# EnterpriseCV-6/Season-NeRF

Measured on AMD Instinct MI355X. Metric: ray-samples/sec (4096 rays x 96 samples forward render, T_NeRF 8x256), higher is better.
Workload: dtype i8x3 (16-bit fixed point as two int8 digits on v_mfma_i32_32x32x32_i8, exact int32 accumulate, fp32 epilogue)

## Files before the change

### season_nerf_amd/csrc/kernels.hip

```cpp
#include "mlp_bf16_device.h"

namespace snerf {


template <int NB, int KS0, int KS1, bool SIN, int TERMS = 3, bool LO_OUT = true>
__device__ __forceinline__ void run_layer(Ring& rg, const uint8_t* stream, uint32_t stream_bytes, lds_char* lds,
                                          lds_cfloat* bias_l, const Frag* in0, const Frag* in1, Frag* out,
                                          f32x16* raw, int wave, int lane) {
    constexpr int KS = KS0 + KS1, NP = NB * KS;
    constexpr bool PIPE = KS >= 4;
    const int h = lane >> 5;
    u32x4 fh[PF], fl[PF] = {};
#pragma unroll
    for (int q = 0; q < PF; ++q) {
        if (q < NP) {
            if (q % kChunkPairs == 0) ring_step(rg, stream, stream_bytes, lds, wave, lane);
            lds_char* ap = lds + rg.cur + (q % kChunkPairs) * kPairBytes + lane * 16;
            fh[q] = *(lds_cu32x4*)ap;
            if (TERMS == 3) fl[q] = *(lds_cu32x4*)(ap + kFragBytes);
        }
    }
    f32x16 accs[2];
    EpiTmp et[8];
    f32x16 next_init = load_bias(bias_l, 0, h);
// ... 113 lines not shown
        const int64_t nc = valid ? n : A.n - 1;
        const int64_t g = VARIANT == 3 ? 0 : nc / A.group_size;

        if constexpr (PROG == PROG_FIELD) {
            float x0, x1, x2;
            if constexpr (VARIANT == 3) raysum_point(rs, A, tile, 4, wave, pass, lane, x0, x1, x2);
            else field_point(A, nc, x0, x1, x2);
            float s0, s1, s2, pcls[C_MAX];
            field_tile_inputs<VARIANT>(A, g, s0, s1, s2, pcls);
            Frag pe[PEPOS_KS];
            make_pe_pos(x0, x1, x2, h, pe);

            constexpr int KW = W / 16, KW2 = W2 / 16;
            Frag hA[KW], hB[KW], x1f[KW2];
            f32x16 raw;
#define LAYER(L, NBv, K0, K1, SINv, IN0, IN1, OUT, RAW)                                                              \
    run_layer<NBv, K0, K1, SINv, (FAST && L != F_FC1) ? 1 : 3, !FAST>(rg, A.stream, A.stream_bytes, lds,                   \
                                 bias_lds + prog_bias_start(PROG_FIELD, W, C_MAX, L), IN0, IN1, OUT, RAW, wave, lane)
            FIELD_TRUNK(LAYER, pe, hA, hB, x1f, raw);
            const float col_r = raw[0], col_g = raw[1], col_b = raw[2], rho_raw = raw[3];
            float sv_raw = 0.f;
            float adj[3 * C_MAX];
#pragma unroll
            for (int i = 0; i < 3 * C_MAX; ++i) adj[i] = 0.f;
            if constexpr (VARIANT <= 1) {
                Frag ps[PESUN_KS];
                make_pe_sun(s0, s1, s2, h, ps);
                Frag sA[KW2], sB[KW2];
                FIELD_SOLAR(LAYER, x1f, ps, sA, sB, raw);
                sv_raw = raw[0];
            }
            if constexpr (VARIANT == 0) {
                FIELD_ADJUST(LAYER, x1f, hA, hB, raw);
#pragma unroll
                for (int i = 0; i < 3 * C_MAX; ++i) adj[i] = raw[i];
            }
#undef LAYER
            if constexpr (VARIANT == 3) {
                RAYSUM_PASS_END(rs, A, tile, pass, passes, 4, wave, wave, 4, true, lane, rho_raw, x0, x1, x2, bias_lds + A.bias_floats);
            } else {
                if (h == 0 && valid) store_field_outputs<VARIANT>(A.out, n, C, x0, x1, x2, col_r, col_g, col_b, rho_raw, sv_raw, adj, pcls);
                tile += gridDim.x;
            }
        } else {
            constexpr int KW = W / 16, W4P = pad32(W / 4), KW4 = W4P / 16;
            f32x16 raw;
#define LAYER(L, NBv, K0, K1, SINv, IN0, IN1, OUT, RAW)                                                              \
    run_layer<NBv, K0, K1, SINv>(rg, A.stream, A.stream_bytes, lds, bias_lds + prog_bias_start(PROG_GROUP, W, C_MAX, L), \
                                 IN0, IN1, OUT, RAW, wave, lane)
            const float t0 = A.time[nc * 4], t1 = A.time[nc * 4 + 1];
            const float s0 = A.sun[nc * 3], s1 = A.sun[nc * 3 + 1], s2 = A.sun[nc * 3 + 2];
            Frag pt[PETIME_KS];
            make_pe_time(t0, t1, h, pt);
            Frag hA[KW], hB[KW];
            LAYER(G_T1, W / 32, PETIME_KS, 0, true, pt, nullptr, hA, nullptr);
            LAYER(G_T2, W / 32, KW, 0, true, hA, nullptr, hB, nullptr);
            LAYER(G_CL, 1, KW, 0, false, hB, nullptr, nullptr, &raw);
            float logit[C_MAX];
#pragma unroll
            for (int c = 0; c < C_MAX; ++c) logit[c] = raw[c];
            Frag ps[PESUN_KS];
            make_pe_sun(s0, s1, s2, h, ps);
            Frag kA[KW4];
            LAYER(G_K1, W4P / 32, PESUN_KS, 0, true, ps, nullptr, kA, nullptr);
            LAYER(G_K2, 1, KW4, 0, false, kA, nullptr, nullptr, &raw);
#undef LAYER
            if (h == 0 && valid) {
                float m = -3.0e38f;
#pragma unroll
                for (int c = 0; c < C_MAX; ++c) if (c < C) m = fmaxf(m, logit[c]);
                float e[C_MAX], sum = 0.f;
#pragma unroll
                for (int c = 0; c < C_MAX; ++c) { e[c] = c < C ? expf(logit[c] - m) : 0.f; sum += e[c]; }
#pragma unroll
                for (int c = 0; c < C_MAX; ++c) if (c < C && A.g_classes) A.g_classes[n * C + c] = e[c] / sum;
#pragma unroll
                for (int k = 0; k < 3; ++k) {
                    if (A.g_sky_raw) A.g_sky_raw[n * 3 + k] = raw[k];
                    if (A.g_sky) A.g_sky[n * 3 + k] = sigmoid_f(raw[k]);
                }
            }
            tile += gridDim.x;
        }
    }
    asm volatile("s_waitcnt vmcnt(0)" ::: "memory");
}

__host__ __device__ constexpr int sun_walk_lds_extra() { return kMaxWalkSuns * 3 * 4; }

__device__ __attribute__((noinline)) void store_softplus(float* p, float x) { *p = softplus_f(x); }

template <int W>
__global__ __launch_bounds__(256, 1) void sun_walk_kernel(const SunWalkArgs SA) {
    const MlpArgs& A = SA.m;
    constexpr int C_MAX = kMaxClasses;
    constexpr int W2 = W / 2;
    const int C = A.n_classes;
    const int n_suns = SA.n_suns;
    FIELD_PROLOGUE(A,
        __attribute__((address_space(3))) float* sun_lds = (__attribute__((address_space(3))) float*)(lds + RING_BYTES + A.bias_floats * 4 + kVoteBytes);
        for (int i = threadIdx.x; i < 3 * n_suns; i += 256) sun_lds[i] = A.sun[i];)

    const int64_t n_tiles = field_tiles(A.n, 0, TILE_PTS, 4);
    snerf_field_out_dev once = A.out;
    once.solar_vis = nullptr;
    once.rho = nullptr;
    for (int64_t tile = blockIdx.x; tile < n_tiles; tile += gridDim.x) {
        const int64_t n = tile * TILE_PTS + wave * 32 + (lane & 31);
        const bool valid = n < A.n;
        const int64_t nc = valid ? n : A.n - 1;
        float x0, x1, x2;
        field_point(A, nc, x0, x1, x2);
        float u0, u1, u2, pcls[C_MAX];
        field_tile_inputs<0>(A, 0, u0, u1, u2, pcls);
        Frag pe[PEPOS_KS];
        make_pe_pos(x0, x1, x2, h, pe);

        constexpr int KW = W / 16, KW2 = W2 / 16;
        Frag hA[KW], hB[KW], x1f[KW2];
        f32x16 raw;
        FIELD_TRUNK(FIELD_LAYER, pe, hA, hB, x1f, raw);
        const float col_r = raw[0], col_g = raw[1], col_b = raw[2], rho_raw = raw[3];
        for (int j = 0; j < n_suns; ++j) {
            const float s0 = sun_lds[3 * j], s1 = sun_lds[3 * j + 1], s2 = sun_lds[3 * j + 2];
            Frag ps[PESUN_KS];
            make_pe_sun(s0, s1, s2, h, ps);
            Frag sA[KW2], sB[KW2];
            FIELD_SOLAR(FIELD_LAYER, x1f, ps, sA, sB, raw);
            if (h == 0 && valid && A.out.solar_vis) A.out.solar_vis[(int64_t)j * A.n + n] = sigmoid_f(raw[0]);
        }
        FIELD_ADJUST(FIELD_LAYER, x1f, hA, hB, raw);
        float adj[3 * C_MAX];
#pragma unroll
        for (int i = 0; i < 3 * C_MAX; ++i) adj[i] = raw[i];
        if (h == 0 && valid) {
            if (A.out.rho) store_softplus(A.out.rho + n, rho_raw);
            store_field_outputs<0>(once, n, C, x0, x1, x2, col_r, col_g, col_b, rho_raw, 0.f, adj, pcls);
        }
    }
    asm volatile("s_waitcnt vmcnt(0)" ::: "memory");
}

__global__ __launch_bounds__(256) void composite_kernel(const CompArgs A) {
    const int lane = threadIdx.x & 63;
    const int64_t r = (int64_t)blockIdx.x * 4 + (threadIdx.x >> 6);
    if (r >= A.n_rays) return;
    const int S = A.n_samples;
    const float tx = A.top[r * 3], ty = A.top[r * 3 + 1], tz = A.top[r * 3 + 2];
    const float bx = A.bot[r * 3], by = A.bot[r * 3 + 1], bz = A.bot[r * 3 + 2];
    const float delta_ray = ray_delta(tx, ty, tz, bx, by, bz, S);
    const bool classic = A.flags & 1, zero_oob = A.flags & 2;
    const float sky0 = A.sky[r * 3], sky1 = A.sky[r * 3 + 1], sky2 = A.sky[r * 3 + 2];

    float carry = 0.f, carry_m = 0.f;
    float a0 = 0.f, a1 = 0.f, a2 = 0.f, svsum = 0.f, acc = 0.f, l0 = 0.f, l1 = 0.f, l2 = 0.f, dist = 0.f;
    float c0 = 0.f, c1 = 0.f, c2 = 0.f;
    float m0 = 0.f, m1 = 0.f, m2 = 0.f;
    float ma0 = 0.f, ma1 = 0.f, ma2 = 0.f;
    for (int base = 0; base < S; base += 64) {
        const int s = base + lane;
        const bool in = s < S;
        const int64_t idx = r * S + (in ? s : S - 1);
        float px, py, pz;
        ray_point(tx, ty, tz, bx, by, bz, A.tvals[in ? s : S - 1], px, py, pz);
        float delta = delta_ray;
        if (zero_oob && outside_cube(px, py, pz)) delta = 0.f;
        const float rho = in ? A.rho[idx] : 0.f;
        const float y = in ? rho * delta : 0.f;
        const RayStep st = transmit_step(y, in, lane, carry);
        carry = st.carry;
        const float pv = st.pv, pe = st.pe, ps = st.ps;
        const float sv = in ? A.solar_vis[idx] : 0.f;
        const float k0 = in ? A.col[idx * 3] : 0.f, k1 = in ? A.col[idx * 3 + 1] : 0.f, k2 = in ? A.col[idx * 3 + 2] : 0.f;
        if (in) {
            if (A.out.pv) A.out.pv[idx] = pv;
            if (A.out.pe) A.out.pe[idx] = pe;
            if (A.out.ps) A.out.ps[idx] = ps;
            if (A.out.delta) A.out.delta[idx] = delta;
        }
        a0 += ps * k0; a1 += ps * k1; a2 += ps * k2;
        svsum += ps * sv;
        acc += ps;
        l0 += ps * px; l1 += ps * py; l2 += ps * pz;
        dist += ps * (delta_ray * (float)(s + 1));
        if (classic) {
            c0 += ps * k0 * (sv + (1.f - sv) * sky0);
            c1 += ps * k1 * (sv + (1.f - sv) * sky1);
            c2 += ps * k2 * (sv + (1.f - sv) * sky2);
        }
        if (A.rho_prior) {
            const float tr = A.trust_dev ? A.trust_dev[0] : A.trust;
            const float rm = in ? (rho * tr + A.rho_prior[idx] * (1.f - tr)) : 0.f;
            const float ym = rm * delta;
            const RayStep stm = transmit_step(ym, in, lane, carry_m);
            carry_m = stm.carry;
            const float psm = stm.ps;
            if (classic) {
                m0 += psm * k0 * (sv + (1.f - sv) * sky0);
                m1 += psm * k1 * (sv + (1.f - sv) * sky1);
                m2 += psm * k2 * (sv + (1.f - sv) * sky2);
                ma0 += psm * k0; ma1 += psm * k1; ma2 += psm * k2;
            } else {
                m0 += psm * k0; m1 += psm * k1; m2 += psm * k2;
            }
        }
    }
    a0 = wave_sum(a0); a1 = wave_sum(a1); a2 = wave_sum(a2);
    svsum = wave_sum(svsum); acc = wave_sum(acc);
    l0 = wave_sum(l0); l1 = wave_sum(l1); l2 = wave_sum(l2); dist = wave_sum(dist);
    if (classic) { c0 = wave_sum(c0); c1 = wave_sum(c1); c2 = wave_sum(c2); }
    if (A.rho_prior) { m0 = wave_sum(m0); m1 = wave_sum(m1); m2 = wave_sum(m2); }
    if (A.rho_prior && classic) { ma0 = wave_sum(ma0); ma1 = wave_sum(ma1); ma2 = wave_sum(ma2); }
    if (lane == 0) {
        const float sv3 = sigmoid_f((svsum - 0.2f) * 30.f);
        const float f0 = sv3 + (1.f - sv3) * sky0, f1 = sv3 + (1.f - sv3) * sky1, f2 = sv3 + (1.f - sv3) * sky2;
        float r0, r1, r2, al0 = a0, al1 = a1, al2 = a2;
        if (A.rho_prior) {
            if (classic) { r0 = m0; r1 = m1; r2 = m2; al0 = ma0; al1 = ma1; al2 = ma2; } else { r0 = m0 * f0; r1 = m1 * f1; r2 = m2 * f2; al0 = m0; al1 = m1; al2 = m2; }
        } else if (classic) { r0 = c0; r1 = c1; r2 = c2; }
        else { r0 = a0 * f0; r1 = a1 * f1; r2 = a2 * f2; }
        if (A.out.rgb) { A.out.rgb[r * 3] = r0; A.out.rgb[r * 3 + 1] = r1; A.out.rgb[r * 3 + 2] = r2; }
        if (A.out.albedo) { A.out.albedo[r * 3] = al0; A.out.albedo[r * 3 + 1] = al1; A.out.albedo[r * 3 + 2] = al2; }
        if (A.out.shadow) A.out.shadow[r] = svsum;
        if (A.out.acc) A.out.acc[r] = acc;
        if (A.out.surf_loc) {
            A.out.surf_loc[r * 3] = l0 / (acc + 1e-8f); A.out.surf_loc[r * 3 + 1] = l1 / (acc + 1e-8f); A.out.surf_loc[r * 3 + 2] = l2 / (acc + 1e-8f);
        }
        if (A.out.surf_dist) A.out.surf_dist[r] = dist / acc;
    }
}

constexpr int T_CHUNK = 12;
__device__ __forceinline__ float sigmoid_fast(float x) { return __builtin_amdgcn_rcpf(1.f + __builtin_amdgcn_exp2f(x * -1.44269504088896341f)); }
template <bool CLASSIC>
__global__ __launch_bounds__(256) void sweep_kernel(const SweepArgs A) {
    constexpr int TH = T_CHUNK / 2;
    const int lane = threadIdx.x & 63, sl = lane & 31, half = lane >> 5;
    const int64_t r = (int64_t)blockIdx.x * 4 + (threadIdx.x >> 6);
    if (r >= A.n_rays) return;
    const int S = A.n_samples, C = A.n_classes;
    const bool explicit_delta = A.deltas != nullptr;
    float tx = 0.f, ty = 0.f, tz = 0.f, bx = 0.f, by = 0.f, bz = 0.f, delta_ray = 0.f;
    if (!explicit_delta) {
        tx = A.top[r * 3]; ty = A.top[r * 3 + 1]; tz = A.top[r * 3 + 2];
        bx = A.bot[r * 3]; by = A.bot[r * 3 + 1]; bz = A.bot[r * 3 + 2];
        const float dx = tx - bx, dy = ty - by, dz = tz - bz;
        delta_ray = __fdiv_rn(__fsqrt_rn(__fadd_rn(__fadd_rn(__fmul_rn(dx, dx), __fmul_rn(dy, dy)), __fmul_rn(dz, dz))), (float)S);
    }
    const bool zero_oob = (A.flags & 2) && !explicit_delta;
    const float sky0 = A.sky[0], sky1 = A.sky[1], sky2 = A.sky[2];
    struct In { float rho, sv, dl, k[3], ad[kMaxClasses][3]; };
    auto fetch = [&](int base) {
        In v;
        const int s = base + sl;
        const int64_t idx = r * S + (s < S ? s : S - 1);
        v.rho = A.rho[idx];
        v.sv = A.solar_vis[idx];
        v.dl = explicit_delta ? A.deltas[idx] : (zero_oob ? A.tvals[s < S ? s : S - 1] : 0.f);
#pragma unroll
        for (int k = 0; k < 3; ++k) v.k[k] = A.col_raw[idx * 3 + k];
        if (A.adjust_vec4 && kMaxClasses >= 4) {
            const float4* p = reinterpret_cast<const float4*>(A.adjust + idx * 12);
            const float4 q0 = p[0], q1 = p[1], q2 = p[2];
            const float f[12] = {q0.x, q0.y, q0.z, q0.w, q1.x, q1.y, q1.z, q1.w, q2.x, q2.y, q2.z, q2.w};
#pragma unroll
            for (int c = 0; c < kMaxClasses; ++c)
#pragma unroll
                for (int k = 0; k < 3; ++k) v.ad[c][k] = c < 4 ? f[c * 3 + k] : 0.f;
            return v;
        }
#pragma unroll
        for (int c = 0; c < kMaxClasses; ++c)
#pragma unroll
            for (int k = 0; k < 3; ++k) v.ad[c][k] = c < C ? A.adjust[(idx * C + c) * 3 + k] : 0.f;
        return v;
    };
    auto half_sum = [](float v) {
#pragma unroll
        for (int o = 16; o > 0; o >>= 1) v += __shfl_xor(v, o, 64);
        return v;
    };
    for (int t0 = 0; t0 < A.n_times; t0 += T_CHUNK) {
        const int tb = t0 + half * TH;
        float cw[TH][kMaxClasses];
#pragma unroll
        for (int t = 0; t < TH; ++t)
#pragma unroll
            for (int c = 0; c < kMaxClasses; ++c) cw[t][c] = (tb + t < A.n_times && c < C) ? A.class_vecs[(tb + t) * C + c] : 0.f;
        float acc[TH][3];
        float accc[CLASSIC ? TH : 1][3];
#pragma unroll
        for (int t = 0; t < TH; ++t) acc[t][0] = acc[t][1] = acc[t][2] = 0.f;
#pragma unroll
        for (int t = 0; t < (CLASSIC ? TH : 1); ++t) accc[t][0] = accc[t][1] = accc[t][2] = 0.f;
        float carry = 0.f, svsum = 0.f, b0 = 0.f, b1 = 0.f, b2 = 0.f;
        In nxt = fetch(0);
        for (int base = 0; base < S; base += 32) {
            const In cur = nxt;
            if (base + 32 < S) nxt = fetch(base + 32);
            const int s = base + sl;
            const bool in = s < S;
            float delta = delta_ray;
            if (explicit_delta) {
                delta = cur.dl;
            } else if (zero_oob) {
                const float tt = cur.dl, omt = __fsub_rn(1.f, tt);
                const float px = __fadd_rn(__fmul_rn(tx, omt), __fmul_rn(bx, tt));
                const float py = __fadd_rn(__fmul_rn(ty, omt), __fmul_rn(by, tt));
                const float pz = __fadd_rn(__fmul_rn(tz, omt), __fmul_rn(bz, tt));
                if (px > 1.f || px < -1.f || py > 1.f || py < -1.f || pz > 1.f || pz < -1.f) delta = 0.f;
            }
            const float y = in ? cur.rho * delta : 0.f;
            float incl = y;
#pragma unroll
            for (int o = 1; o < 32; o <<= 1) {
                const float t = __shfl_up(incl, o, 32);
                if (sl >= o) incl += t;
            }
            const float below = __shfl_up(incl, 1, 32);
            const float excl = carry + (sl == 0 ? 0.f : below);
            carry += __shfl(incl, 31, 32);
            const float ps = in ? expf(-excl) * (1.f - expf(-y)) : 0.f;
            const float sv = in ? cur.sv : 0.f;
            svsum += ps * sv;
            const float k0 = cur.k[0], k1 = cur.k[1], k2 = cur.k[2];
            b0 += ps * sigmoid_fast(k0); b1 += ps * sigmoid_fast(k1); b2 += ps * sigmoid_fast(k2);
#pragma unroll
            for (int t = 0; t < TH; ++t) {
                float m0 = 0.f, m1 = 0.f, m2 = 0.f;
#pragma unroll
                for (int c = 0; c < kMaxClasses; ++c) { m0 += cw[t][c] * cur.ad[c][0]; m1 += cw[t][c] * cur.ad[c][1]; m2 += cw[t][c] * cur.ad[c][2]; }
                const float q0 = ps * sigmoid_fast(k0 + m0), q1 = ps * sigmoid_fast(k1 + m1), q2 = ps * sigmoid_fast(k2 + m2);
                acc[t][0] += q0; acc[t][1] += q1; acc[t][2] += q2;
                if constexpr (CLASSIC) {
                    accc[t][0] += q0 * (sv + (1.f - sv) * sky0);
                    accc[t][1] += q1 * (sv + (1.f - sv) * sky1);
                    accc[t][2] += q2 * (sv + (1.f - sv) * sky2);
                }
            }
        }
        svsum = half_sum(svsum);
        b0 = half_sum(b0); b1 = half_sum(b1); b2 = half_sum(b2);
        const float mask = sigmoid_f((svsum - 0.2f) * 30.f);
        const float f0 = mask + (1.f - mask) * sky0, f1 = mask + (1.f - mask) * sky1, f2 = mask + (1.f - mask) * sky2;
#pragma unroll
        for (int t = 0; t < TH; ++t) {
            const float v0 = half_sum(acc[t][0]), v1 = half_sum(acc[t][1]), v2 = half_sum(acc[t][2]);
            float c0 = 0.f, c1 = 0.f, c2 = 0.f;
            if constexpr (CLASSIC) { c0 = half_sum(accc[t][0]); c1 = half_sum(accc[t][1]); c2 = half_sum(accc[t][2]); }
            if (sl == 0 && tb + t < A.n_times) {
                const int64_t o = ((int64_t)(tb + t) * A.n_rays + r) * 3;
                if (A.season) { A.season[o] = v0; A.season[o + 1] = v1; A.season[o + 2] = v2; }
                if (A.shaded) { A.shaded[o] = v0 * f0; A.shaded[o + 1] = v1 * f1; A.shaded[o + 2] = v2 * f2; }
                if constexpr (CLASSIC) { A.classic[o] = c0; A.classic[o + 1] = c1; A.classic[o + 2] = c2; }
            }
        }
        if (lane == 0 && t0 == 0) {
            if (A.raw_shadow) A.raw_shadow[r] = svsum;
            if (A.shadow_adjust) { A.shadow_adjust[r * 3] = f0; A.shadow_adjust[r * 3 + 1] = f1; A.shadow_adjust[r * 3 + 2] = f2; }
            if (A.base) { A.base[r * 3] = b0; A.base[r * 3 + 1] = b1; A.base[r * 3 + 2] = b2; }
        }
    }
}

hipError_t launch_sweep(const SweepArgs& a, hipStream_t st) {
// ... 426 lines not shown
```

### season_nerf_amd/csrc/kernels_i8x2.hip

```cpp
#include <type_traits>

#include "mlp_i8_device.h"

namespace snerf {

constexpr int NW2 = 8;
constexpr int TILE2 = 32 * NW2;
constexpr int DMA_WAVES2 = 4, PIECES4 = kChunkBytes / kFragBytes / DMA_WAVES2;
constexpr int RING2_D = 7;
constexpr int PFX = 2;
static_assert(PIECES4 == 4 && kChunkPairs == 8, "dma_chunk4 moves four pieces per loading wave; barrier positions assume 8-pair chunks");

struct Ring2 {
    uint32_t wr;
    uint32_t goff;
    uint32_t cur;
};
__device__ __forceinline__ uint32_t ring2_next(uint32_t off) {
    off += kChunkBytes;
    return off == RING2_D * kChunkBytes ? 0u : off;
}
__device__ __forceinline__ void dma_chunk4(const uint8_t* stream, uint32_t goff, lds_char* lds, uint32_t wr, int wave, int lane) {
    const uint8_t* b0 = stream + goff + wave * (4 * kFragBytes);
    const uint32_t dst = (uint32_t)(uintptr_t)(lds + wr + wave * (4 * kFragBytes));
    const uint32_t voff = lane * 16;
    uint32_t keep;
    asm volatile(
        "s_mov_b32 %0, m0\n\t"
        "s_mov_b32 m0, %2\n\t"
        "s_nop 0\n\t"
        "global_load_lds_dwordx4 %1, %3\n\t"
        "s_add_u32 m0, m0, 0x400\n\t"
        "s_nop 0\n\t"
        "global_load_lds_dwordx4 %1, %4\n\t"
        "s_add_u32 m0, m0, 0x400\n\t"
        "s_nop 0\n\t"
        "global_load_lds_dwordx4 %1, %5\n\t"
        "s_add_u32 m0, m0, 0x400\n\t"
        "s_nop 0\n\t"
        "global_load_lds_dwordx4 %1, %6\n\t"
        "s_mov_b32 m0, %0"
        : "=&s"(keep)
        : "v"(voff), "s"(dst), "s"(b0), "s"(b0 + kFragBytes), "s"(b0 + 2 * kFragBytes), "s"(b0 + 3 * kFragBytes)
        : "memory", "scc");
}

template <int PHASE>
__device__ __forceinline__ void ring_step2(Ring2& rg, const uint8_t* stream, uint32_t stream_bytes, lds_char* lds, int wave, int lane) {
#if defined(SNERF_ABLATE) && (ABL & 4)
    return;
#endif
    if (PHASE == 0) {
        asm volatile("s_waitcnt vmcnt(%0)\n\ts_barrier" ::"n"((RING2_D - 3) * PIECES4) : "memory");
        dma_chunk4(stream, rg.goff, lds, rg.wr, wave, lane);
    } else {
        asm volatile("s_barrier" ::: "memory");
    }
    rg.goff += kChunkBytes;
    if (rg.goff >= stream_bytes) rg.goff = 0;
    rg.wr = ring2_next(rg.wr);
}

struct TabQ {
    f32x4 sc, bi;
};
__device__ __forceinline__ TabQ load_tab_quad(lds_cfloat* tab_l, int b, int h, int g) {
    typedef volatile const __attribute__((address_space(3))) f32x4 lds_vf32x4;
    lds_vf32x4* tp = (lds_vf32x4*)(tab_l + (b * 2 + h) * 32);
    TabQ t;
    t.sc = tp[g];
    t.bi = tp[4 + g];
    return t;
}
__device__ __forceinline__ TabQ load_tab_quad_h(lds_cfloat* tab_h, int b, int g) {
    typedef volatile const __attribute__((address_space(3))) f32x4 lds_vf32x4;
    lds_vf32x4* tp = (lds_vf32x4*)(tab_h + b * 64);
    TabQ t;
    t.sc = tp[g];
    t.bi = tp[4 + g];
    return t;
}
template <int TAB_, int NB_, bool SIN_, bool RAWL_, bool DEP_>
struct Carry {
    static constexpr bool on = true, SIN = SIN_, RAWL = RAWL_, DEP = DEP_;
    static constexpr int TAB = TAB_, NB = NB_;
};
struct NoCarry {
    static constexpr bool on = false, SIN = false, RAWL = false, DEP = false;
    static constexpr int TAB = 0, NB = 1;
};
__host__ __device__ constexpr bool carry_fits(int nb, bool dep) { return !dep || nb >= 2; }
struct CarryDst {
    Frag8* out;
    f32x16* raw;
    const float* rawx;
};

struct Boundary {
    int m[16];
    i32x4 fT[PFX], fL[PFX];
};

template <bool SIN, bool RAWL>
__device__ __forceinline__ void epi_quad(const int* m, int g, const TabQ& t, const f32x4* rqg, const float* rawx, Frag8* ob, f32x16* raw) {
    float v[4];
#if defined(SNERF_ABLATE) && (ABL & 16)
#pragma unroll
    for (int j = 0; j < 4; ++j) v[j] = __builtin_bit_cast(float, (m[4 * g + j] & 0x007fffff) | 0x3f000000) - 0.75f;
#else
#pragma unroll
    for (int j = 0; j < 4; ++j) v[j] = __builtin_fmaf((float)m[4 * g + j], t.sc[j], t.bi[j]);
    if constexpr (RAWL) {
#pragma unroll
        for (int j = 0; j < 4; ++j)
            v[j] = __builtin_fmaf(rqg[0][j], rawx[0], __builtin_fmaf(rqg[1][j], rawx[1], __builtin_fmaf(rqg[2][j], rawx[2], v[j])));
    }
#endif
    if constexpr (SIN) {
#if defined(SNERF_ABLATE) && (ABL & 8)
#pragma unroll
        for (int j = 0; j < 4; ++j) v[j] = __builtin_fmaf(__builtin_amdgcn_fractf(v[j]), 2.f, -1.f);
#elif !(defined(SNERF_ABLATE) && (ABL & 16))
#pragma unroll
        for (int j = 0; j < 4; ++j) v[j] = sin2pi(v[j]);
#endif
        int hi, lo;
        digits4(v[0], v[1], v[2], v[3], hi, lo);
        asm volatile("" : "+v"(hi), "+v"(lo));
        ob->hi[g] = hi;
        ob->lo[g] = lo;
    } else {
#pragma unroll
        for (int j = 0; j < 4; ++j) (*raw)[4 * g + j] = v[j];
    }
}

__host__ __device__ constexpr bool field_feeds_next(int l) { return l != F_HEAD && l != F_S4; }
static_assert(F_S1 == F_HEAD + 1 && F_A1 == F_S4 + 1 && F_FC1 == 0, "the kernels' LAYER macros build the carry of layer L from layer L - 1");
__host__ __device__ constexpr int field_last(int variant) { return variant == 0 ? F_AC : variant == 1 ? F_S4 : F_HEAD; }
__host__ __device__ constexpr bool field_carries(int W, int variant, int C, int l) {
    return l != field_last(variant) && carry_fits(prog_layer(PROG_FIELD, W, C, l, FMT_I8).n_out / 32, field_feeds_next(l));
}

#if defined(SNERF_ABLATE) && (ABL & 2)
constexpr bool kNoFragReads = true;
#else
constexpr bool kNoFragReads = false;
#endif
#define REQUEST(QN, SLOT)                                                                              \
    do {                                                                                               \
        if ((QN) % kChunkPairs == 0) {                                                                 \
            ring_step2<PHASE>(rg, stream, stream_bytes, lds, wave, lane);                              \
            if ((QN) > 0) rg.cur = ring2_next(rg.cur);                                                 \
        }                                                                                              \
        lds_char* ap_ = lds + rg.cur + ((QN) % kChunkPairs) * kPairBytes + lane * 16;                  \
        if (!kNoFragReads) {                                                                           \
            fT[SLOT] = *(lds_ci32x4*)ap_;                                                              \
            fL[SLOT] = *(lds_ci32x4*)(ap_ + kFragBytes);                                               \
        } else {                                                                                       \
            asm volatile("" : "+v"(fT[SLOT]), "+v"(fL[SLOT]));                                         \
        }                                                                                              \
    } while (0)
#define REQUEST_NEXT(J, SLOT)                                                                          \
    do {                                                                                               \
        if ((J) == 0) {                                                                                \
            ring_step2<PHASE>(rg, stream, stream_bytes, lds, wave, lane);                              \
            rg.cur = ring2_next(rg.cur);                                                               \
        }                                                                                              \
        lds_char* ap_ = lds + rg.cur + (J) * kPairBytes + lane * 16;                                   \
        if (!kNoFragReads) {                                                                           \
            fT[SLOT] = *(lds_ci32x4*)ap_;                                                              \
            fL[SLOT] = *(lds_ci32x4*)(ap_ + kFragBytes);                                               \
        } else {                                                                                       \
            asm volatile("" : "+v"(fT[SLOT]), "+v"(fL[SLOT]));                                         \
        }                                                                                              \
    } while (0)

template <int NB, int KS0, int KS1, bool SIN, bool RAWL = false, int PHASE = 0, bool OPQ = false, class PEND = NoCarry, bool HANDOFF = false, bool PRE_IN = false,
          bool PRE_OUT = false>
__device__ __forceinline__ void run_layer8x2(Ring2& rg, const uint8_t* stream, uint32_t stream_bytes, lds_char* lds, lds_cfloat* tab0, lds_cfloat* tab_l,
                                             const Frag8* in0, const Frag8* in1, Frag8* out, f32x16* raw, Boundary& bd, const CarryDst& pd,
                                             int wave, int lane, const float* rawx = nullptr) {
    constexpr int KS = KS0 + KS1, NP = NB * KS;
    constexpr int NBP = PEND::NB;
    static_assert(!PRE_OUT || (NP >= PFX && NP % PFX == 0), "the successor expects its pair j in fragment slot j");
    static_assert(!PRE_IN || NP >= PFX, "the predecessor requested PFX pairs of this layer");
    int (&m)[16] = bd.m;
    i32x4 (&fT)[PFX] = bd.fT;
    i32x4 (&fL)[PFX] = bd.fL;
    static_assert(!PEND::on || carry_fits(NBP, PEND::DEP), "a carried block that is the operand of k-step 0 has no k-step to run in");
    static_assert(!(PEND::on && PEND::DEP) || NBP <= KS0, "Carry::DEP: the producer's output is in0");
    typedef volatile const __attribute__((address_space(3))) f32x4 lds_vf32x4;
    f32x4 rq[4][3];
    const int h = lane >> 5;
    lds_cfloat* ptab_l = tab0 + PEND::TAB;
    lds_cfloat* base_h = (PEND::on ? ptab_l : tab_l) + 32 * h;
    if constexpr (OPQ) asm volatile("" : "+v"(base_h));
// ... 136 lines not shown
#pragma unroll
        for (int j = 0; j < 4; ++j) raw[4 * cg + j] = v[j];
    }
}

template <int NB, int KS0, int KS1, bool SIN, bool RAWL = false, int PHASE = 0, class PEND = NoCarry, bool HANDOFF = false, bool PRE_IN = false,
          bool PRE_OUT = false>
__device__ __forceinline__ void run_layer16(Ring2& rg, const uint8_t* stream, uint32_t stream_bytes, lds_char* lds, lds_cfloat* tab0, lds_cfloat* tab_l,
                                            const FragK* in0, const FragK* in1, FragK* out, float* raw, BoundaryK& bd, const CarryDstK& pd,
                                            int wave, int lane, const float (*rawx)[3] = nullptr) {
    constexpr int KS = KS0 + KS1, NP = NB * KS;
    constexpr int NBP = PEND::NB;
    static_assert(!PRE_OUT || (NP >= PFX && NP % PFX == 0), "the successor expects its pair j in fragment slot j");
    static_assert(!PRE_IN || NP >= PFX, "the predecessor requested PFX pairs of this layer");
    static_assert(!PEND::on || carry_fits_k64(NBP, PEND::DEP), "a carried block that is an operand of k-step 0 has no k-step to run in");
    static_assert(!(PEND::on && PEND::DEP) || NBP == 4 * KS0, "Carry::DEP: the producer's output is in0");
    int (&m)[8] = bd.m;
    i32x4 (&fT)[PFX] = bd.fT;
    i32x4 (&fL)[PFX] = bd.fL;
    typedef volatile const __attribute__((address_space(3))) f32x4 lds_vf32x4;
    int g = lane >> 4;
    asm volatile("" : "+v"(g));
    lds_cfloat* ptab_l = tab0 + PEND::TAB;
    lds_cfloat* lo_l = PEND::on ? ptab_l : tab_l;
    lds_cfloat* base_g = lo_l + 8 * g;
    lds_cfloat* rbase_g = lo_l + 12 * g;
    const int d_own = (int)(tab_l - lo_l);
    auto tabq = [&](int b_) {
        lds_vf32x4* tp = (lds_vf32x4*)(base_g + d_own + b_ * 32);
        TabQ t;
        t.sc = tp[0];
        t.bi = tp[1];
        return t;
    };
    auto ptabq = [&]() {
        lds_vf32x4* tp = (lds_vf32x4*)(base_g + (NBP - 1) * 32);
        TabQ t;
        t.sc = tp[0];
        t.bi = tp[1];
        return t;
    };
    f32x4 rq[3];
    auto load_rq = [&](int b_of) {
        if constexpr (RAWL) {
            lds_vf32x4* tp = (lds_vf32x4*)(rbase_g + d_own + 2 * 16 * NB + b_of * 48);
            rq[0] = tp[0]; rq[1] = tp[1]; rq[2] = tp[2];
        }
    };
    auto load_prq = [&]() {
        if constexpr (PEND::RAWL) {
            lds_vf32x4* tp = (lds_vf32x4*)(rbase_g + 2 * 16 * NBP + (NBP - 1) * 48);
            rq[0] = tp[0]; rq[1] = tp[1]; rq[2] = tp[2];
        }
    };
    if constexpr (kNoFragReads) {
#pragma unroll
        for (int q = 0; q < PFX; ++q) { fT[q] = i32x4{lane, 1, 2, 3}; fL[q] = i32x4{4, lane, 6, 7}; }
    }
    if constexpr (!PRE_IN) {
#pragma unroll
        for (int q = 0; q < PFX; ++q) {
            if (q < NP) REQUEST(q, q);
        }
    }
    AccK acc;
    TabQ tq;
    auto quad = [&](int cg, int b_of) { epi_quad_k64<SIN, RAWL>(m, cg, tq, rq, rawx, out + b_of / 4, b_of % 4, raw); };
    auto pquad = [&](int cg) { epi_quad_k64<PEND::SIN, PEND::RAWL>(m, cg, tq, rq, pd.rawx, pd.out + (NBP - 1) / 4, (NBP - 1) % 4, pd.raw); };
    auto slot = [](int cg, bool carried) constexpr { return carried && PEND::DEP ? (cg * ((NBP - 1) / 4) * 2) / 3 : (cg * KS) / 2; };
#pragma unroll
    for (int b = 0; b < NB; ++b) {
        const bool carried = b == 0;
        if (b > 0 || PEND::on) {
            if (b > 0) {
                tq = tabq(b - 1);
                load_rq(b - 1);
#pragma unroll
                for (int i = 0; i < 8; ++i) m[i] = (int)(((uint32_t)acc.M[i >> 2][i & 3] << 8) + (uint32_t)acc.X[i >> 2][i & 3]);
            } else {
                tq = ptabq();
                load_prq();
            }
            asm volatile("" ::: "memory");
            __builtin_amdgcn_sched_barrier(0);
        }
#pragma unroll
        for (int cg = 0; cg < 2; ++cg)
#pragma unroll
            for (int i = 0; i < 4; ++i) { acc.M[cg][i] = 0; acc.X[cg][i] = 0; }
#pragma unroll
        for (int s = 0; s < KS; ++s) {
            const int q = b * KS + s;
            const i32x4 aT = fT[q % PFX], aL = fL[q % PFX];
            if (((s + PHASE) & 1) == 0) __builtin_amdgcn_s_setprio(0); else __builtin_amdgcn_s_setprio(3);
            if (q + PFX < NP) REQUEST(q + PFX, q % PFX);
            else if constexpr (PRE_OUT) REQUEST_NEXT(q + PFX - NP, q % PFX);
            mfma_k64x3(aT, aL, s < KS0 ? in0[s] : in1[s - KS0], acc);
            if (b > 0 || PEND::on) {
#pragma unroll
                for (int cg = 0; cg < 2; ++cg)
                    if (slot(cg, carried) == s) {
                        if (b > 0) quad(cg, b - 1);
                        else pquad(cg);
                    }
            }
            asm volatile("" ::: "memory");
            __builtin_amdgcn_sched_barrier(0);
        }
    }
#pragma unroll
    for (int i = 0; i < 8; ++i) m[i] = (int)(((uint32_t)acc.M[i >> 2][i & 3] << 8) + (uint32_t)acc.X[i >> 2][i & 3]);
    if constexpr (HANDOFF) {
        asm volatile("" ::: "memory");
        __builtin_amdgcn_sched_barrier(0);
    } else {
        asm volatile("" ::: "memory");
        tq = tabq(NB - 1);
        load_rq(NB - 1);
#pragma unroll
        for (int cg = 0; cg < 2; ++cg) {
            quad(cg, NB - 1);
            asm volatile("" ::: "memory");
            __builtin_amdgcn_sched_barrier(0);
        }
    }
    if constexpr (!PRE_OUT) rg.cur = ring2_next(rg.cur);
}
#undef REQUEST
#undef REQUEST_NEXT

__host__ __device__ constexpr bool k64_built(int W) { return W == 256; }
bool i8x2_k64_built(int W, int variant) { return variant >= 0 && variant <= 3 && k64_built(W); }

template <int W, int VARIANT, int PHASE>
__device__ __forceinline__ void field_tiles2(const MlpArgs& A, Ring2& rg, lds_char* lds, __attribute__((address_space(3))) float* tab_lds,
                                             int wave, int lane);
template <int W, int VARIANT, int PHASE>
__device__ __forceinline__ void field_tiles16(const MlpArgs& A, Ring2& rg, lds_char* lds, __attribute__((address_space(3))) float* tab_lds,
                                              int wave, int lane);

template <int W, int VARIANT>
__global__ __launch_bounds__(64 * NW2, 1) void mlp_i8x2_kernel(const MlpArgs A) {
    extern __shared__ __attribute__((aligned(16))) char smem[];
    constexpr int C_MAX = kMaxClasses;
    constexpr int W2 = W / 2;
    lds_char* lds = (lds_char*)smem;
    __attribute__((address_space(3))) float* tab_lds = (__attribute__((address_space(3))) float*)(lds + RING2_D * kChunkBytes);

    const int lane = threadIdx.x & 63;
    const int wave = __builtin_amdgcn_readfirstlane(threadIdx.x >> 6);
    const int h = lane >> 5;
    const int C = A.n_classes;

    for (int i = threadIdx.x; i < A.bias_floats; i += 64 * NW2) tab_lds[i] = A.bias[i];

    Ring2 rg;
    rg.cur = 0;
    rg.goff = 0;
    {
        uint32_t wr = 0;
#pragma unroll
        for (int c = 0; c < RING2_D - 2; ++c) {
            if (wave < DMA_WAVES2) dma_chunk4(A.stream, rg.goff, lds, wr, wave, lane);
            rg.goff += kChunkBytes;
            if (rg.goff >= A.stream_bytes) rg.goff = 0;
            wr += kChunkBytes;
        }
        rg.wr = wr;
    }
    __syncthreads();

    bool k64 = false;
    if constexpr (k64_built(W)) k64 = A.k64 != 0;
    if (k64) {
        if constexpr (k64_built(W)) {
            if (wave < 4) field_tiles16<W, VARIANT, 0>(A, rg, lds, tab_lds, wave, lane);
            else field_tiles16<W, VARIANT, 1>(A, rg, lds, tab_lds, wave, lane);
        }
    } else {
        if (wave < 4) field_tiles2<W, VARIANT, 0>(A, rg, lds, tab_lds, wave, lane);
        else field_tiles2<W, VARIANT, 1>(A, rg, lds, tab_lds, wave, lane);
    }
    asm volatile("s_waitcnt vmcnt(0)" ::: "memory");
}

template <int W, int VARIANT, int PHASE>
__device__ __forceinline__ void field_tiles16(const MlpArgs& A, Ring2& rg, lds_char* lds, __attribute__((address_space(3))) float* tab_lds,
                                              int wave, int lane) {
    constexpr int C_MAX = kMaxClasses;
    constexpr int W2 = W / 2;
    const int h = lane >> 5, gq = lane >> 4;
    const int C = A.n_classes;
    const int64_t n_tiles = field_tiles(A.n, VARIANT, TILE2, NW2);
    const int passes = VARIANT == 3 ? (A.n_samples + 31) / 32 : 1;
    int pass = 0;
    RaySum rs;
    for (int64_t tile = blockIdx.x; tile < n_tiles;) {
        const int64_t n = tile * TILE2 + wave * 32 + (lane & 31);
        const bool valid = n < A.n;
        const int64_t nc = valid ? n : A.n - 1;
        const int64_t g = VARIANT == 3 ? 0 : nc / A.group_size;

        float x0, x1, x2;
        if constexpr (VARIANT == 3) raysum_point(rs, A, tile, NW2, wave, pass, lane, x0, x1, x2);
        else field_point(A, nc, x0, x1, x2);
        float s0, s1, s2, pcls[C_MAX];
        field_tile_inputs<VARIANT>(A, g, s0, s1, s2, pcls);
        float rx_p[2][3], rx_s[2][3];
        k64_two_points(x0, x1, x2, lane, rx_p);
        FragK pe;
        make_pe_pos_k64(rx_p, gq, pe);

        constexpr int KW = W / 64, KW2 = W2 / 64;
        FragK hA[KW], hB[KW];
        float raw[8];
        BoundaryK bd;
#define SHAPE(L) k64_layer(W, C_MAX, L)
#define TAB(L) k64_table_start(W, C_MAX, L)
#define HAND(L) (L >= F_FC1 && field_carries_k64(W, VARIANT, C_MAX, L))
#define PEND_T(P) std::conditional_t<HAND(P), Carry<TAB(P), k64_blocks(SHAPE(P)), layer_sine(SHAPE(P)), layer_reads_raw(SHAPE(P)), field_feeds_next(P)>, NoCarry>
#define LAYER(L, IN0, IN1, OUT, RAW, RX, PO, PR, PX)                                                                                                 \
    run_layer16<k64_blocks(SHAPE(L)), SHAPE(L).ks0, SHAPE(L).ks1, layer_sine(SHAPE(L)), layer_reads_raw(SHAPE(L)), PHASE, PEND_T(L - 1), HAND(L),   \
                L != F_FC1, L != field_last(VARIANT)>(rg, A.stream, A.stream_bytes, lds, tab_lds, tab_lds + TAB(L), IN0, IN1, OUT, RAW, bd,         \
                                                      (CarryDstK{PO, PR, PX}), wave, lane, RX)
        FragK x1f[KW2];
        I8_TRUNK(LAYER, &pe, hA, hB, x1f, raw, rx_p,
                 if constexpr (VARIANT != 3) {
                     const bool up = (lane & 16) != 0;
                     x0 = up ? rx_p[1][0] : rx_p[0][0]; x1 = up ? rx_p[1][1] : rx_p[0][1]; x2 = up ? rx_p[1][2] : rx_p[0][2];
                 });
        float col_r, col_g, col_b, rho_raw;
        float sv_raw = 0.f;
        float adj[3 * C_MAX];
#pragma unroll
        for (int i = 0; i < 3 * C_MAX; ++i) adj[i] = 0.f;
#define HEAD_OUT() col_r = k64_head_row(raw, 0, lane), col_g = k64_head_row(raw, 1, lane), col_b = k64_head_row(raw, 2, lane), rho_raw = k64_head_row(raw, 3, lane)
        if constexpr (VARIANT <= 1) {
            k64_two_points(s0, s1, s2, lane, rx_s);
            FragK ps;
            make_pe_sun_k64(rx_s, gq, ps);
            FragK sA[KW2], sB[KW2];
            I8_SOLAR(LAYER, x1f, &ps, sA, sB, raw, rx_s, HEAD_OUT(););
            if constexpr (VARIANT == 1) sv_raw = k64_head_row(raw, 0, lane);
        } else {
            HEAD_OUT();
        }
        if constexpr (VARIANT == 0) {
            I8_ADJUST(LAYER, x1f, hA, hB, raw, sv_raw = k64_head_row(raw, 0, lane););
#pragma unroll
            for (int i = 0; i < 3 * C_MAX; ++i) adj[i] = k64_head_row(raw, i, lane);
        }
#undef HEAD_OUT
#undef LAYER
#undef PEND_T
#undef HAND
#undef TAB
#undef SHAPE
        if constexpr (VARIANT == 3) {
            RAYSUM_PASS_END(rs, A, tile, pass, passes, NW2, wave, wave, NW2, true, lane, rho_raw, x0, x1, x2, tab_lds + A.bias_floats);
        } else {
            if (h == 0 && valid) store_field_outputs<VARIANT>(A.out, n, C, x0, x1, x2, col_r, col_g, col_b, rho_raw, sv_raw, adj, pcls);
            tile += gridDim.x;
        }
    }
    __builtin_amdgcn_s_setprio(0);
}

template <int W, int VARIANT, int PHASE>
__device__ __forceinline__ void field_tiles2(const MlpArgs& A, Ring2& rg, lds_char* lds, __attribute__((address_space(3))) float* tab_lds,
                                             int wave, int lane) {
    constexpr int C_MAX = kMaxClasses;
    constexpr int W2 = W / 2;
    const int h = lane >> 5;
    const int C = A.n_classes;
    const int64_t n_tiles = field_tiles(A.n, VARIANT, TILE2, NW2);
    const int passes = VARIANT == 3 ? (A.n_samples + 31) / 32 : 1;
    int pass = 0;
    RaySum rs;
    for (int64_t tile = blockIdx.x; tile < n_tiles;) {
        const int64_t n = tile * TILE2 + wave * 32 + (lane & 31);
        const bool valid = n < A.n;
        const int64_t nc = valid ? n : A.n - 1;
        const int64_t g = VARIANT == 3 ? 0 : nc / A.group_size;

        float x0, x1, x2;
        if constexpr (VARIANT == 3) raysum_point(rs, A, tile, NW2, wave, pass, lane, x0, x1, x2);
        else field_point(A, nc, x0, x1, x2);
        float s0, s1, s2, pcls[C_MAX];
        field_tile_inputs<VARIANT>(A, g, s0, s1, s2, pcls);
        Frag8 pe[PEPOS_KS8];
        make_pe_pos8<VARIANT == 3>(x0, x1, x2, h, pe);

        constexpr int KW = W / 32, KW2 = W2 / 32;
        Frag8 hA[KW], hB[KW];
        f32x16 raw;
        Boundary bd;
#define SHAPE(L) field_layer(W, C_MAX, L, FMT_I8)
#define TAB(L) prog_table_start(PROG_FIELD, W, C_MAX, L)
#define HAND(L) (L >= F_FC1 && field_carries(W, VARIANT, C_MAX, L))
#define PEND_T(P) std::conditional_t<HAND(P), Carry<TAB(P), SHAPE(P).nb(), layer_sine(SHAPE(P)), layer_reads_raw(SHAPE(P)), field_feeds_next(P)>, NoCarry>
        constexpr bool XPF = KW2 >= PFX && KW2 % PFX == 0;
#define LAYER(L, IN0, IN1, OUT, RAW, RX, PO, PR, PX)                                                                                                 \
    run_layer8x2<SHAPE(L).nb(), SHAPE(L).ks0, SHAPE(L).ks1, layer_sine(SHAPE(L)), layer_reads_raw(SHAPE(L)), PHASE, VARIANT == 3, PEND_T(L - 1), HAND(L), \
                 XPF && L != F_FC1, XPF && L != field_last(VARIANT)>(rg, A.stream, A.stream_bytes, lds, tab_lds, tab_lds + TAB(L), IN0, IN1, OUT, RAW, bd, \
                                                                     (CarryDst{PO, PR, PX}), wave, lane, RX)
        const float rx_p[3] = {x0, x1, x2}, rx_s[3] = {s0, s1, s2};
        Frag8 x1f[KW2];
        I8_TRUNK(LAYER, pe, hA, hB, x1f, &raw, rx_p);
        float col_r, col_g, col_b, rho_raw;
        float sv_raw = 0.f;
        float adj[3 * C_MAX];
#pragma unroll
        for (int i = 0; i < 3 * C_MAX; ++i) adj[i] = 0.f;
        if constexpr (VARIANT <= 1) {
            Frag8 ps[PESUN_KS8];
            make_pe_sun8(s0, s1, s2, h, ps);
            Frag8 sA[KW2], sB[KW2];
            I8_SOLAR(LAYER, x1f, ps, sA, sB, &raw, rx_s, col_r = raw[0], col_g = raw[1], col_b = raw[2], rho_raw = raw[3];);
            if constexpr (VARIANT == 1) sv_raw = raw[0];
        } else {
            col_r = raw[0], col_g = raw[1], col_b = raw[2], rho_raw = raw[3];
        }
// ... 42 lines not shown
```

Before: 571.5 million.

## Prefetch composite inputs, skip unused reductions, DMA bias table into LDS

The composite kernel now fetches the next 64-sample chunk of inputs one iteration ahead, so global loads overlap with the scan arithmetic. Accumulations and wave reductions whose outputs are not requested are skipped. In the MLP kernel, the bias table is copied into LDS with global_load_lds DMA pieces instead of a per-thread copy loop, with a scalar tail for leftovers. A full vmcnt(0) wait is added before the barrier, which makes the warm-up ring loads drain there too.

```diff
diff --git a/season_nerf_amd/csrc/kernels.hip b/season_nerf_amd/csrc/kernels.hip
--- a/season_nerf_amd/csrc/kernels.hip
+++ b/season_nerf_amd/csrc/kernels.hip
@@ -289,26 +289,53 @@
     const bool classic = A.flags & 1, zero_oob = A.flags & 2;
     const float sky0 = A.sky[r * 3], sky1 = A.sky[r * 3 + 1], sky2 = A.sky[r * 3 + 2];
 
+    const bool has_prior = A.rho_prior != nullptr;
+    const bool want_loc = A.out.surf_loc != nullptr, want_dist = A.out.surf_dist != nullptr;
+    const bool want_acc = A.out.acc || want_loc || want_dist;
+    const bool want_sv = A.out.shadow || (A.out.rgb && !classic);
+    const bool want_a = !has_prior && (A.out.albedo || (A.out.rgb && !classic));
+    const bool want_c = classic && !has_prior && A.out.rgb;
+
+    struct In { float t, rho, sv, k0, k1, k2, rp; };
+    auto fetch = [&](int base) {
+        In v;
+        const int s = base + lane;
+        const bool in = s < S;
+        const int64_t idx = r * S + (in ? s : S - 1);
+        const float t = A.tvals[in ? s : S - 1], rho = A.rho[idx], sv = A.solar_vis[idx];
+        const float k0 = A.col[idx * 3], k1 = A.col[idx * 3 + 1], k2 = A.col[idx * 3 + 2];
+        const float rp = has_prior ? A.rho_prior[idx] : 0.f;
+        v.t = t;
+        v.rho = in ? rho : 0.f;
+        v.sv = in ? sv : 0.f;
+        v.k0 = in ? k0 : 0.f; v.k1 = in ? k1 : 0.f; v.k2 = in ? k2 : 0.f;
+        v.rp = in ? rp : 0.f;
+        return v;
+    };
+
     float carry = 0.f, carry_m = 0.f;
     float a0 = 0.f, a1 = 0.f, a2 = 0.f, svsum = 0.f, acc = 0.f, l0 = 0.f, l1 = 0.f, l2 = 0.f, dist = 0.f;
     float c0 = 0.f, c1 = 0.f, c2 = 0.f;
     float m0 = 0.f, m1 = 0.f, m2 = 0.f;
     float ma0 = 0.f, ma1 = 0.f, ma2 = 0.f;
+    In nxt = fetch(0);
     for (int base = 0; base < S; base += 64) {
+        const In cur = nxt;
+        if (base + 64 < S) nxt = fetch(base + 64);
         const int s = base + lane;
         const bool in = s < S;
         const int64_t idx = r * S + (in ? s : S - 1);
         float px, py, pz;
-        ray_point(tx, ty, tz, bx, by, bz, A.tvals[in ? s : S - 1], px, py, pz);
+        ray_point(tx, ty, tz, bx, by, bz, cur.t, px, py, pz);
         float delta = delta_ray;
         if (zero_oob && outside_cube(px, py, pz)) delta = 0.f;
-        const float rho = in ? A.rho[idx] : 0.f;
+        const float rho = cur.rho;
         const float y = in ? rho * delta : 0.f;
         const RayStep st = transmit_step(y, in, lane, carry);
         carry = st.carry;
         const float pv = st.pv, pe = st.pe, ps = st.ps;
-        const float sv = in ? A.solar_vis[idx] : 0.f;
-        const float k0 = in ? A.col[idx * 3] : 0.f, k1 = in ? A.col[idx * 3 + 1] : 0.f, k2 = in ? A.col[idx * 3 + 2] : 0.f;
+        const float sv = cur.sv;
+        const float k0 = cur.k0, k1 = cur.k1, k2 = cur.k2;
         if (in) {
             if (A.out.pv) A.out.pv[idx] = pv;
             if (A.out.pe) A.out.pe[idx] = pe;
@@ -317,17 +344,17 @@
         }
         a0 += ps * k0; a1 += ps * k1; a2 += ps * k2;
         svsum += ps * sv;
-        acc += ps;
-        l0 += ps * px; l1 += ps * py; l2 += ps * pz;
-        dist += ps * (delta_ray * (float)(s + 1));
-        if (classic) {
+        if (want_acc) acc += ps;
+        if (want_loc) { l0 += ps * px; l1 += ps * py; l2 += ps * pz; }
+        if (want_dist) dist += ps * (delta_ray * (float)(s + 1));
+        if (want_c) {
             c0 += ps * k0 * (sv + (1.f - sv) * sky0);
             c1 += ps * k1 * (sv + (1.f - sv) * sky1);
             c2 += ps * k2 * (sv + (1.f - sv) * sky2);
         }
-        if (A.rho_prior) {
+        if (has_prior) {
             const float tr = A.trust_dev ? A.trust_dev[0] : A.trust;
-            const float rm = in ? (rho * tr + A.rho_prior[idx] * (1.f - tr)) : 0.f;
+            const float rm = in ? (rho * tr + cur.rp * (1.f - tr)) : 0.f;
             const float ym = rm * delta;
             const RayStep stm = transmit_step(ym, in, lane, carry_m);
             carry_m = stm.carry;
@@ -342,12 +369,14 @@
             }
         }
     }
-    a0 = wave_sum(a0); a1 = wave_sum(a1); a2 = wave_sum(a2);
-    svsum = wave_sum(svsum); acc = wave_sum(acc);
-    l0 = wave_sum(l0); l1 = wave_sum(l1); l2 = wave_sum(l2); dist = wave_sum(dist);
-    if (classic) { c0 = wave_sum(c0); c1 = wave_sum(c1); c2 = wave_sum(c2); }
-    if (A.rho_prior) { m0 = wave_sum(m0); m1 = wave_sum(m1); m2 = wave_sum(m2); }
-    if (A.rho_prior && classic) { ma0 = wave_sum(ma0); ma1 = wave_sum(ma1); ma2 = wave_sum(ma2); }
+    if (want_a) { a0 = wave_sum(a0); a1 = wave_sum(a1); a2 = wave_sum(a2); }
+    if (want_sv) svsum = wave_sum(svsum);
+    if (want_acc) acc = wave_sum(acc);
+    if (want_loc) { l0 = wave_sum(l0); l1 = wave_sum(l1); l2 = wave_sum(l2); }
+    if (want_dist) dist = wave_sum(dist);
+    if (want_c) { c0 = wave_sum(c0); c1 = wave_sum(c1); c2 = wave_sum(c2); }
+    if (has_prior) { m0 = wave_sum(m0); m1 = wave_sum(m1); m2 = wave_sum(m2); }
+    if (has_prior && classic) { ma0 = wave_sum(ma0); ma1 = wave_sum(ma1); ma2 = wave_sum(ma2); }
     if (lane == 0) {
         const float sv3 = sigmoid_f((svsum - 0.2f) * 30.f);
         const float f0 = sv3 + (1.f - sv3) * sky0, f1 = sv3 + (1.f - sv3) * sky1, f2 = sv3 + (1.f - sv3) * sky2;
diff --git a/season_nerf_amd/csrc/kernels_i8x2.hip b/season_nerf_amd/csrc/kernels_i8x2.hip
--- a/season_nerf_amd/csrc/kernels_i8x2.hip
+++ b/season_nerf_amd/csrc/kernels_i8x2.hip
@@ -43,6 +43,21 @@
         : "=&s"(keep)
         : "v"(voff), "s"(dst), "s"(b0), "s"(b0 + kFragBytes), "s"(b0 + 2 * kFragBytes), "s"(b0 + 3 * kFragBytes)
         : "memory", "scc");
+}
+
+__device__ __forceinline__ void dma_piece(const uint8_t* src, lds_char* lds, uint32_t off, int lane) {
+    const uint32_t dst = (uint32_t)(uintptr_t)(lds + off);
+    const uint32_t voff = lane * 16;
+    uint32_t keep;
+    asm volatile(
+        "s_mov_b32 %0, m0\n\t"
+        "s_mov_b32 m0, %2\n\t"
+        "s_nop 0\n\t"
+        "global_load_lds_dwordx4 %1, %3\n\t"
+        "s_mov_b32 m0, %0"
+        : "=&s"(keep)
+        : "v"(voff), "s"(dst), "s"(src)
+        : "memory");
 }
 
 template <int PHASE>
@@ -485,8 +500,6 @@
     const int h = lane >> 5;
     const int C = A.n_classes;
 
-    for (int i = threadIdx.x; i < A.bias_floats; i += 64 * NW2) tab_lds[i] = A.bias[i];
-
     Ring2 rg;
     rg.cur = 0;
     rg.goff = 0;
@@ -501,6 +514,17 @@
         }
         rg.wr = wr;
     }
+    {
+        int moved = 0;
+        if (((uintptr_t)A.bias & 15) == 0) {
+            const int pieces = A.bias_floats * 4 / kFragBytes;
+            for (int p = wave; p < pieces; p += NW2)
+                dma_piece((const uint8_t*)A.bias + (size_t)p * kFragBytes, lds, RING2_D * kChunkBytes + p * kFragBytes, lane);
+            moved = pieces * (kFragBytes / 4);
+        }
+        for (int i = moved + threadIdx.x; i < A.bias_floats; i += 64 * NW2) tab_lds[i] = A.bias[i];
+    }
+    asm volatile("s_waitcnt vmcnt(0)" ::: "memory");
     __syncthreads();
 
     bool k64 = false;
```

Result: no change. 571.9 million, median of 5 (+0.1%).
